# djene-mengistu/UAPS

Measured on AMD Instinct MI355X. Metric: training images/sec (labeled+unlabeled) NEU-Seg 256x256 K=3, higher is better.
Workload: dtype f32

## Files before the change

### uaps_amd/csrc/mid_bwd_row.hip

```cpp
#include "../../include/uaps_hip.h"
#include "conv_kernels.hpp"
#include "conv_split.hpp"
#include "hints.hpp"
#include "row_pieces.hpp"

extern "C" int uaps_conv_get_mode(void);
extern "C" unsigned uaps_conv_get_tuning(void);

namespace uaps {

struct MidBwdArgs {
    const float* dact;
    const float* y2;
    const float* coef;
    float dt_slope;
    int dt_Bg;
    const float* y1;
    const float2* xf;
    float slope;
    int Bg;
    const float* wp;
    const float* wscale;
    int CGP;
    float* g;
    float* slab; float* bslab; int nsplit;
    const float* dy_bound; const float* in_bound;
    float dy_mul, in_mul;
    const float* bs_mean; const float* bs_invstd; const float* bs_gamma; const float* bs_beta;
    float2* partials;
    float* bs_max;
    unsigned* err;
    int B, H;
};

__global__ __launch_bounds__(512, 2) void mid_bwd_row_kernel(MidBwdArgs a) {
    using G = RowGeom<16>;
    constexpr int NG = G::NG, ROWS = G::ROWS, CI = G::CI, NTHR = 512, NXL = G::NXL, MW = G::MW, D_UNITS = G::D_UNITS;
    constexpr int RED_FLOATS = 2 * 10 * 256;
    static_assert(RED_FLOATS / 4 <= G::X_UNITS, "the reduction scratch fits the input image");

    __shared__ __attribute__((aligned(16))) u32x4 sX[G::X_UNITS];
    __shared__ __attribute__((aligned(16))) u32x4 sD[2 * D_UNITS];
    __shared__ __attribute__((aligned(16))) u32x4 sIn[2 * G::PIECE];
    __shared__ __attribute__((aligned(16))) float sG[16 * G::GS];

    const f32x2 sd = h16_scale(__builtin_fmaxf(bound_of(a.dy_bound, a.dy_mul), 0.f));
    const f32x2 sx = h16_scale(__builtin_fmaxf(bound_of(a.in_bound, a.in_mul), 0.f));
    const float sc_d = sd.x, inv_d = sd.y, sc_x = sx.x, inv_x = sx.y;

    const int tid = threadIdx.x, lane = tid & 63, wave = tid >> 6;
    const int j = lane & 15, kq = lane >> 4;
    const int wave_u = __builtin_amdgcn_readfirstlane(wave);
    const int HW = a.H * G::WIDTH;
    const uint32_t HW4 = (uint32_t)HW * 4u;

    RowRuns rr;
    if (!row_runs<G>(a.B, a.H, a.nsplit, rr)) return;

    zero_x_halo<G, NTHR>(sX, tid);
    zero_ring_margins<G, NTHR>(sIn, tid);

    float bs_md = 0.f, bs_mx = 0.f;

    if (wave_u < 4) {
        const int sp = wave_u;
        const int dc0 = wave_u * 4, cg = wave_u >> 1, ch = wave_u & 1;
        const bool want_bias = a.bslab != nullptr;
        f32x4 rd[4], ry[4];
        bool d_in = false;
        float dtc[4][6];
        auto load_d = [&](int b, int gy, f32x4 (&dd)[4], f32x4 (&yy)[4], bool& ok) {
            ok = load_rows4<G>(a.dact, b, gy, a.H, dc0, lane, dd);
            load_rows4<G>(a.y2, b, gy, a.H, dc0, lane, yy);
        };
        auto store_d = [&](f32x4 (&dd)[4], f32x4 (&yy)[4], bool ok, int slot, int buf) {
            f32x4 v[4];
#pragma unroll
            for (int i = 0; i < 4; ++i) {
                asm volatile("" : "+v"(dd[i]));
                asm volatile("" : "+v"(yy[i]));
#pragma unroll
                for (int k = 0; k < 4; ++k) {
                    const float g0 = dd[i][k];
                    const float yc = yy[i][k] - dtc[i][0];
                    const float z = yc * dtc[i][2] + dtc[i][3];
                    const float d = z > 0.f ? g0 : g0 * a.dt_slope;
                    const float t = dtc[i][2] * (d - dtc[i][4] - (yc * dtc[i][1]) * dtc[i][5]);
                    v[i][k] = ok ? t : 0.f;
                }
            }
            store_ring_rows<G>(sIn, v, sc_d, cg, ch, lane, slot);
            if (buf >= 0) {
#pragma unroll
                for (int i = 0; i < 4; ++i) {
                    unsigned a0, a1, b0, b1;
                    conv_split2h(v[i][0] * sc_d, v[i][1] * sc_d, a0, a1);
                    conv_split2h(v[i][2] * sc_d, v[i][3] * sc_d, b0, b1);
                    const int c = dc0 + i;
                    *reinterpret_cast<uint2*>(reinterpret_cast<unsigned*>(&sD[buf * D_UNITS + c * NG]) + lane * 2) = make_uint2(a0, b0);
                    *reinterpret_cast<uint2*>(reinterpret_cast<unsigned*>(&sD[buf * D_UNITS + (16 + c) * NG]) + lane * 2) = make_uint2(a1, b1);
                }
            }
        };

        f32x4 acc[9];
        f32x4 accb = f32x4{0.f, 0.f, 0.f, 0.f};
#pragma unroll
        for (int t = 0; t < 9; ++t) acc[t] = f32x4{0.f, 0.f, 0.f, 0.f};

        for (int run = rr.begin; run < rr.end; ++run) {
            const int b = run / rr.rpi, r0 = (run % rr.rpi) * ROWS;
            const int grp2 = b / a.dt_Bg;
#pragma unroll
            for (int i = 0; i < 4; ++i)
#pragma unroll
                for (int k = 0; k < 6; ++k) dtc[i][k] = a.coef[((size_t)grp2 * 16 + dc0 + i) * 8 + k];
            {
                f32x4 da[4], ya[4], db[4], yb[4];
                bool oka, okb;
                load_d(b, r0 - 1, da, ya, oka);
                load_d(b, r0, db, yb, okb);
                load_d(b, r0 + 1, rd, ry, d_in);
                __builtin_amdgcn_sched_barrier(0);
                store_d(da, ya, oka, 0, -1);
                store_d(db, yb, okb, 1, 0);
                store_d(rd, ry, d_in, 2, 1);
            }
            __syncthreads();
            int s0 = 0, buf = 0;
#pragma unroll 1
            for (int t = r0; t < r0 + ROWS; ++t) {
                const bool more = t + 1 < r0 + ROWS;
                if (more) load_d(b, t + 2, rd, ry, d_in);
                int s1, s2;
                ring_slots<G>(s0, s1, s2);
                const auto slot_of = [&](int ky) { return ky == 0 ? s0 : (ky == 1 ? s1 : s2); };
                const u32x4* sDb = sD + buf * D_UNITS;
#pragma unroll
                for (int sgi = 0; sgi < 2; ++sgi) {
                    const int gq = (sp * 2 + sgi) * 4 + kq;
                    f16x8 af[2];
                    read_dy_frag<G>(sDb, j, gq, af);
                    tap_contract<G>(sX, af, j, gq, slot_of, want_bias, acc, accb);
                }
                __syncthreads();
                if (more) store_d(rd, ry, d_in, s0, buf);
                s0 = s1; buf ^= 1;
                __syncthreads();
            }
        }

        ksplit_reduce<1>(reinterpret_cast<float*>(sX), sp, 0, lane, acc, accb);
        if (sp == 0) store_slabs<true>(a.slab, a.bslab, want_bias, rr.split, 16, CI, 0, j, kq, acc, accb, inv_d, inv_x, a.err);
    } else {
        const int wg = wave_u - 4;
        const int xc0 = wg * NXL;
        const float out_scale_a = inv_d, out_scale_w = a.wscale[1];

        GradFrags<G> wf;
        load_grad_frags<G, 16>(wf, a.wp, a.CGP, j, j, kq, wg * MW);

        f32x4 rx[NXL], xa[NXL], xb[NXL];
        BnRowSums<G> bn;
        bool x_in = false;
        auto store_x = [&](f32x4 (&src)[NXL], bool ok, int slot) { store_act_rows<G>(sX, src, bn.cf, ok, a.slope, sc_x, xc0, lane, slot); };

        for (int run = rr.begin; run < rr.end; ++run) {
            const int b = run / rr.rpi, r0 = (run % rr.rpi) * ROWS;
            bn_run_begin(bn, a.xf, a.bs_mean, a.bs_invstd, a.bs_gamma, a.bs_beta, b / a.Bg, xc0);
            {
                f32x4 ra[NXL];
                const bool oka = load_rows4<G>(a.y1, b, r0 - 1, a.H, xc0, lane, ra);
                const bool okb = load_rows4<G>(a.y1, b, r0, a.H, xc0, lane, xa);
                x_in = load_rows4<G>(a.y1, b, r0 + 1, a.H, xc0, lane, xb);
                __builtin_amdgcn_sched_barrier(0);
                store_x(ra, oka, 0);
                store_x(xa, okb, 1);
                store_x(xb, x_in, 2);
            }
            __syncthreads();
            int s0 = 0;
            const __amdgpu_buffer_rsrc_t rs_g = make_rsrc(a.g + (size_t)b * CI * HW, (uint32_t)CI * HW4);
#pragma unroll 1
            for (int t = r0; t < r0 + ROWS; ++t) {
                const bool more = t + 1 < r0 + ROWS;
                if (more) x_in = load_rows4<G>(a.y1, b, t + 2, a.H, xc0, lane, rx);
                int s1, s2;
                ring_slots<G>(s0, s1, s2);

                f32x4 gacc[MW];
#pragma unroll
                for (int m = 0; m < MW; ++m) gacc[m] = f32x4{0.f, 0.f, 0.f, 0.f};
                grad_row_tiles<G>(sIn, wf, s0, s1, s2, gacc);
                put_grad_row<G>(sG, gacc, out_scale_a, out_scale_w, j, kq, wg * MW, a.err);
                __syncthreads();

#pragma unroll
                for (int i = 0; i < NXL; ++i) bn_row(bn, i, take_row_out<G>(sG, rs_g, xc0 + i, t, HW, lane), xa[i], a.slope, bs_md, bs_mx);
                if (more) store_x(rx, x_in, s0);
#pragma unroll
                for (int i = 0; i < NXL; ++i) { xa[i] = xb[i]; xb[i] = rx[i]; }
                s0 = s1;
                __syncthreads();
            }
            bn_run_end(bn, a.partials, a.B, b, rr.rpi, r0 / ROWS, xc0, lane);
        }
        __syncthreads(); __syncthreads(); __syncthreads(); __syncthreads();
    }
    block_amax_to(a.bs_max, bs_md, sG);
    block_amax_to(a.bs_max + UAPS_BOUND_FLOATS, bs_mx, sG + 16);
}

}

extern "C" int uaps_mid_bwd_fused(const float* dact, const float* y2, const float* coef, float slope2, int groups2, const float* y1,
                                  const void* xf, float slope, int groups, const float* wb, const float* dy_bound, float dy_mul,
                                  const float* x_bound, float x_mul, const float* save_mean, const float* save_invstd,
                                  const float* gamma, const float* beta, int want_bias, int B, int Cin, int Cout, int H, int W, int ks,
                                  int cfg, float* g, void* partials, float* maxes, void* ws, size_t ws_bytes, uaps_stream_t stream) {
    if (!dact || !y1 || !xf || !wb || !save_mean || !save_invstd || !gamma || !beta || !g || !partials || !maxes || !ws) return UAPS_EINVAL;
    if (B <= 0 || Cin <= 0 || Cout <= 0 || H <= 0 || W <= 0 || groups < 1 || B % groups || (uintptr_t)xf % 8) return UAPS_EINVAL;
    if ((y2 || coef) && (!y2 || !coef || groups2 < 1 || B % groups2)) return UAPS_EINVAL;
    if (!(slope >= 0.f && slope <= 1.f)) return UAPS_ERANGE;
    if (ks != 3 || Cin != 16 || Cout != 16 || W != 256 || H % 16 || H > 65536 || (cfg & ~0x3ff)) return UAPS_ENOFORM;
    if (!y2 || !coef) return UAPS_ENOFORM;
    if (uaps_conv_get_mode() != 2 || !dy_bound || !x_bound) return UAPS_ENOFORM;
    if (uaps_conv_get_tuning() & (UAPS_TUNE_NO_ROW_WRW | UAPS_TUNE_NO_SPLIT_WRW)) return UAPS_ENOFORM;
    if (((uintptr_t)dact | (uintptr_t)y2 | (uintptr_t)y1 | (uintptr_t)g | (uintptr_t)wb | (uintptr_t)ws | (uintptr_t)coef) % 16) return UAPS_ENOFORM;
    uaps::MidBwdArgs a{};
    const int rc = uaps::row_wrw_bn_args(a, 16, B, Cin, Cout, H, W, ks, cfg, want_bias, ws, ws_bytes, dy_bound, dy_mul, x_bound, x_mul,
                                         save_mean, save_invstd, gamma, beta, partials, maxes);
    if (rc) return rc;
    uaps::account_bytes(4.0 * B * H * W * (3.0 * Cout + 1.0 * Cin));
    a.dact = dact; a.y2 = y2; a.coef = coef; a.dt_slope = slope2; a.dt_Bg = B / groups2;
    a.y1 = y1; a.xf = (const float2*)xf; a.slope = slope; a.Bg = B / groups;
    const uaps::H16BwdWeights w16 = uaps::h16_bwd_weights(wb, Cin, Cout);
    a.wp = w16.wp; a.wscale = w16.wscale; a.CGP = w16.CGP;
    a.g = g;
    a.B = B; a.H = H;
    UAPS_LAUNCH_MAIN(uaps::mid_bwd_row_kernel, dim3(uaps::row_grid(a.nsplit)), dim3(512), 0, (hipStream_t)stream, a);
    return (int)hipGetLastError();
}
```

### uaps_amd/csrc/row_pieces.hpp

```cpp
#pragma once
#include "conv_kernels.hpp"
#include "conv_split.hpp"
#include "hints.hpp"

namespace uaps {

template <int CI_>
struct RowGeom {
    static constexpr int WIDTH = 256, ROWS = 16, NSLOT = 3, CI = CI_;
    static constexpr int NG = WIDTH / 8, XG = NG + 2;
    static constexpr int X_UNITS = 2 * CI * NSLOT * XG;
    static constexpr int D_UNITS = 2 * 16 * NG;
    static constexpr int IW = WIDTH + 8, CGU = NSLOT * IW, PIECE = 2 * CGU, XS = 3;
    static constexpr int NQ = 9 * 2, NSTEP = (NQ + 3) / 4, MW = 4;
    static constexpr int GS = WIDTH + 4;
    static constexpr int NXL = 4;
};

struct RowRuns { int split, rpi, begin, end; };
template <class G>
__device__ __forceinline__ bool row_runs(int B, int H, int nsplit, RowRuns& r) {
    r.split = xcd_swizzle(blockIdx.x, gridDim.x);
    if (r.split >= nsplit) return false;
    r.rpi = H / G::ROWS;
    const int nruns = B * r.rpi;
    r.begin = (int)((long)nruns * r.split / nsplit); r.end = (int)((long)nruns * (r.split + 1) / nsplit);
    return true;
}
template <class G>
__device__ __forceinline__ void ring_slots(int s0, int& s1, int& s2) {
    s1 = s0 + 1 >= G::NSLOT ? s0 + 1 - G::NSLOT : s0 + 1; s2 = s1 + 1 >= G::NSLOT ? s1 + 1 - G::NSLOT : s1 + 1;
}
template <class G, int NTHR>
__device__ __forceinline__ void zero_x_halo(u32x4* sX, int tid) {
    for (int e = tid; e < 2 * G::CI * G::NSLOT * 2; e += NTHR) sX[(e / 2) * G::XG + (e % 2) * (G::XG - 1)] = u32x4{0u, 0u, 0u, 0u};
}
template <class G, int NTHR>
__device__ __forceinline__ void zero_ring_margins(u32x4* sIn, int tid) {
    for (int e = tid; e < 2 * 2 * G::NSLOT * 8; e += NTHR) sIn[(e / 8) * G::IW + (e % 8 < 4 ? e % 8 : G::IW - 8 + e % 8)] = u32x4{0u, 0u, 0u, 0u};
}

template <class G>
__device__ __forceinline__ bool load_rows4(const float* t, int b, int gy, int H, int c0, int lane, f32x4 (&dst)[4]) {
    const int HW = H * G::WIDTH;
    const uint32_t HW4 = (uint32_t)HW * 4u;
    const bool ok = (unsigned)gy < (unsigned)H;
    const __amdgpu_buffer_rsrc_t rs = make_rsrc(t + (size_t)b * 16 * HW, 16u * HW4);
    const uint32_t off = (uint32_t)(c0 * HW + gy * G::WIDTH + lane * 4) * 4u;
#pragma unroll
    for (int i = 0; i < 4; ++i) dst[i] = __builtin_bit_cast(f32x4, __builtin_amdgcn_raw_buffer_load_b128(rs, (int)(ok ? off + (uint32_t)i * HW4 : kOob), 0, 0));
    return ok;
}

template <class G, class SlotOf>
__device__ __forceinline__ void tap_contract(const u32x4* sX, const f16x8 (&af)[2], int ci, int gq, const SlotOf& slot_of, bool bias,
                                             f32x4 (&acc)[9], f32x4& accb) {
    constexpr unsigned kOnes = 0x3C003C00u;
    const f16x8 ones = __builtin_bit_cast(f16x8, u32x4{kOnes, kOnes, kOnes, kOnes});
    if (bias) {
        accb = __builtin_amdgcn_mfma_f32_16x16x32_f16(af[1], ones, accb, 0, 0, 0);
        accb = __builtin_amdgcn_mfma_f32_16x16x32_f16(af[0], ones, accb, 0, 0, 0);
    }
#pragma unroll
    for (int ky = 0; ky < 3; ++ky) {
        const int slot = slot_of(ky);
        f16x8 bf[3][2];
#pragma unroll
        for (int p = 0; p < 2; ++p) {
            const int u = ((p * G::CI + ci) * G::NSLOT + slot) * G::XG + gq + 1;
            const u32x4 c = sX[u];
            const unsigned cl3 = reinterpret_cast<const unsigned*>(&sX[u - 1])[3];
            const unsigned cr0 = reinterpret_cast<const unsigned*>(&sX[u + 1])[0];
            const unsigned t01 = __builtin_amdgcn_alignbit(c[1], c[0], 16), t12 = __builtin_amdgcn_alignbit(c[2], c[1], 16);
            const unsigned t23 = __builtin_amdgcn_alignbit(c[3], c[2], 16);
            const unsigned tE0 = __builtin_amdgcn_alignbit(c[0], cl3, 16), t3E = __builtin_amdgcn_alignbit(cr0, c[3], 16);
            bf[0][p] = __builtin_bit_cast(f16x8, u32x4{tE0, t01, t12, t23});
            bf[1][p] = __builtin_bit_cast(f16x8, c);
            bf[2][p] = __builtin_bit_cast(f16x8, u32x4{t01, t12, t23, t3E});
        }
#pragma unroll
        for (int kx = 0; kx < 3; ++kx) {
            f32x4 c = acc[ky * 3 + kx];
            c = __builtin_amdgcn_mfma_f32_16x16x32_f16(af[1], bf[kx][0], c, 0, 0, 0);
            c = __builtin_amdgcn_mfma_f32_16x16x32_f16(af[0], bf[kx][1], c, 0, 0, 0);
            c = __builtin_amdgcn_mfma_f32_16x16x32_f16(af[0], bf[kx][0], c, 0, 0, 0);
            acc[ky * 3 + kx] = c;
        }
    }
}
template <class G>
__device__ __forceinline__ void read_dy_frag(const u32x4* sD, int j, int gq, f16x8 (&af)[2]) {
#pragma unroll
    for (int p = 0; p < 2; ++p) af[p] = __builtin_bit_cast(f16x8, sD[(p * 16 + j) * G::NG + gq]);
}

template <int WCI>
__device__ __forceinline__ void ksplit_reduce(float* red, int sp, int wci, int lane, f32x4 (&acc)[9], f32x4& accb) {
#pragma unroll
    for (int s = 2; s >= 1; s >>= 1) {
        if (sp >= s && sp < 2 * s) {
            float* p = red + (size_t)((sp - s) * WCI + wci) * 10 * 256 + lane;
#pragma unroll
            for (int t = 0; t < 9; ++t)
#pragma unroll
                for (int r = 0; r < 4; ++r) p[(t * 4 + r) * 64] = acc[t][r];
#pragma unroll
            for (int r = 0; r < 4; ++r) p[(36 + r) * 64] = accb[r];
        }
        __syncthreads();
        if (sp < s) {
            const float* p = red + (size_t)(sp * WCI + wci) * 10 * 256 + lane;
#pragma unroll
            for (int t = 0; t < 9; ++t)
#pragma unroll
                for (int r = 0; r < 4; ++r) acc[t][r] += p[(t * 4 + r) * 64];
#pragma unroll
            for (int r = 0; r < 4; ++r) accb[r] += p[(36 + r) * 64];
        }
        __syncthreads();
    }
}

template <bool PIN = false>
__device__ __forceinline__ void store_slabs(float* slab, float* bslab, bool bias, int split, int CoutS, int CinS, int ci0, int j, int kq,
                                            const f32x4 (&acc)[9], const f32x4& accb, float inv_d, float inv_x, unsigned* err) {
    slab += (size_t)split * 9 * CoutS * CinS;
    float chk = 0.f;
    const float inv = inv_d * inv_x;
#pragma unroll
    for (int t = 0; t < 9; ++t) {
        note_nonfinite(chk, acc[t]);
#pragma unroll
        for (int r = 0; r < 4; ++r) {
            const int co = kq * 4 + r, ci = ci0 + j;
            if (co < CoutS && ci < CinS) slab[((size_t)t * CoutS + co) * CinS + ci] = acc[t][r] * inv;
        }
    }
    report_nonfinite(err, chk, UAPS_ERR_WRW_NONFINITE);
    if (bias && j == 0) {
        float inv_b = inv_d;
        if constexpr (PIN) asm volatile("" : "+v"(inv_b));
#pragma unroll
        for (int r = 0; r < 4; ++r)
            if (kq * 4 + r < CoutS) bslab[(size_t)split * CoutS + kq * 4 + r] = accb[r] * inv_b;
    }
}

template <class G>
struct BnRowSums {
    f32x2 cf[G::NXL];
    float mu[G::NXL], is[G::NXL], sc[G::NXL], sh[G::NXL];
    float st_s[G::NXL][4], st_q[G::NXL][4];
};

template <class G>
__device__ __forceinline__ void store_act_rows(u32x4* sX, f32x4 (&src)[G::NXL], const f32x2 (&cf)[G::NXL], bool ok, float slope, float sc_x,
                                               int xc0, int lane, int slot) {
#pragma unroll
    for (int i = 0; i < G::NXL; ++i) {
        asm volatile("" : "+v"(src[i]));
        float v[4];
#pragma unroll
        for (int k = 0; k < 4; ++k) {
            const float z = __builtin_fmaf(src[i][k], cf[i].x, cf[i].y);
            v[k] = ok ? __builtin_fmaxf(z, z * slope) : 0.f;
        }
        unsigned a0, a1, b0, b1;
        conv_split2h(v[0] * sc_x, v[1] * sc_x, a0, a1);
        conv_split2h(v[2] * sc_x, v[3] * sc_x, b0, b1);
        const int c = xc0 + i;
        unsigned* p0 = reinterpret_cast<unsigned*>(&sX[(c * G::NSLOT + slot) * G::XG + 1]) + lane * 2;
        unsigned* p1 = reinterpret_cast<unsigned*>(&sX[((G::CI + c) * G::NSLOT + slot) * G::XG + 1]) + lane * 2;
        *reinterpret_cast<uint2*>(p0) = make_uint2(a0, b0);
        *reinterpret_cast<uint2*>(p1) = make_uint2(a1, b1);
    }
}

template <class G>
__device__ __forceinline__ void store_ring_rows(u32x4* sIn, const f32x4 (&v)[4], float scale, int cg, int ch, int lane, int slot) {
    const int base = (cg * G::NSLOT + slot) * G::IW + 4 + lane * 4;
#pragma unroll
    for (int k = 0; k < 4; ++k) {
        unsigned q00, q01, q10, q11;
        conv_split2h(v[0][k] * scale, v[1][k] * scale, q00, q01);
        conv_split2h(v[2][k] * scale, v[3][k] * scale, q10, q11);
        *reinterpret_cast<uint2*>(reinterpret_cast<unsigned*>(&sIn[base + k]) + ch * 2) = make_uint2(q00, q10);
        *reinterpret_cast<uint2*>(reinterpret_cast<unsigned*>(&sIn[G::PIECE + base + k]) + ch * 2) = make_uint2(q01, q11);
    }
}

template <class G>
struct GradFrags {
    u32x4 bfr[G::NSTEP][2];
    int kxo[G::NSTEP], kyv[G::NSTEP], abase[G::MW];
};
template <class G, int CoutP>
__device__ __forceinline__ void load_grad_frags(GradFrags<G>& f, const float* wp, int CGP, int co, int j, int kq, int tile0) {
    const __amdgpu_buffer_rsrc_t rs_w = make_rsrc(wp, (uint32_t)(2 * 9) * CGP * CoutP * 16u);
#pragma unroll
    for (int s = 0; s < G::NSTEP; ++s) {
        const int q = 4 * s + kq, tap = q / 2, cgq = q % 2;
#pragma unroll
        for (int p = 0; p < 2; ++p) {
            const uint32_t off = q < G::NQ ? (uint32_t)(((p * 9 + tap) * CGP + cgq) * CoutP + co) * 16u : kOob;
            f.bfr[s][p] = __builtin_amdgcn_raw_buffer_load_b128(rs_w, (int)off, 0, 0);
        }
        const int qq = q < G::NQ ? q : 0;
        f.kxo[s] = (qq % 2) * G::CGU + (qq / 2) % 3; f.kyv[s] = (qq / 2) / 3;
    }
#pragma unroll
    for (int m = 0; m < G::MW; ++m) f.abase[m] = (tile0 + m) * 16 + j + G::XS;
}

template <class G>
__device__ __forceinline__ void grad_row_tiles(const u32x4* sIn, const GradFrags<G>& f, int s0, int s1, int s2, f32x4 (&gacc)[G::MW]) {
    constexpr int NSTEP = G::NSTEP, MW = G::MW;
    int aoff[NSTEP];
#pragma unroll
    for (int s = 0; s < NSTEP; ++s) aoff[s] = f.kxo[s] + (f.kyv[s] == 0 ? s0 : (f.kyv[s] == 1 ? s1 : s2)) * G::IW;
    constexpr int NUN = NSTEP * MW;
    u32x4 af[2][2];
    auto read_a = [&](int u, u32x4 (&dst)[2]) {
        const int s = u / MW, m = u % MW;
#pragma unroll
        for (int p = 0; p < 2; ++p) dst[p] = sIn[p * G::PIECE + f.abase[m] + aoff[s]];
    };
    read_a(0, af[0]);
#pragma unroll
    for (int u = 0; u < NUN; ++u) {
        const int s = u / MW, m = u % MW;
        if (u + 1 < NUN) read_a(u + 1, af[(u + 1) & 1]);
        const auto Hf = [](const u32x4& v) { return __builtin_bit_cast(f16x8, v); };
        f32x4 c = gacc[m];
        c = __builtin_amdgcn_mfma_f32_16x16x32_f16(Hf(af[u & 1][1]), Hf(f.bfr[s][0]), c, 0, 0, 0);
        c = __builtin_amdgcn_mfma_f32_16x16x32_f16(Hf(af[u & 1][0]), Hf(f.bfr[s][1]), c, 0, 0, 0);
        c = __builtin_amdgcn_mfma_f32_16x16x32_f16(Hf(af[u & 1][0]), Hf(f.bfr[s][0]), c, 0, 0, 0);
        gacc[m] = c;
        if (u + 1 < NUN) __builtin_amdgcn_sched_group_barrier(0x100, 2, 0);
        __builtin_amdgcn_sched_group_barrier(0x008, 3, 0);
    }
}
template <class G>
__device__ __forceinline__ void put_grad_row(float* sG, const f32x4 (&gacc)[G::MW], float out_scale_a, float out_scale_w, int j, int kq,
                                             int tile0, unsigned* err) {
    float chk = 0.f;
#pragma unroll
    for (int m = 0; m < G::MW; ++m) {
        f32x4 v = gacc[m];
        v *= out_scale_a; v *= out_scale_w;
        v += 0.f;
        note_nonfinite(chk, v);
        *reinterpret_cast<f32x4*>(&sG[j * G::GS + (tile0 + m) * 16 + kq * 4]) = v;
    }
    report_nonfinite(err, chk, UAPS_ERR_CONV_NONFINITE);
}
template <class G>
__device__ __forceinline__ f32x4 take_row_out(const float* sG, __amdgpu_buffer_rsrc_t rs_g, int c, int t, int HW, int lane) {
    const f32x4 gv = *reinterpret_cast<const f32x4*>(&sG[c * G::GS + lane * 4]);
    __builtin_amdgcn_raw_buffer_store_b128(__builtin_bit_cast(u32x4, gv), rs_g, (int)((uint32_t)(c * HW + t * G::WIDTH + lane * 4) * 4u), 0, 0);
    return gv;
}

template <class G>
__device__ __forceinline__ void bn_run_begin(BnRowSums<G>& s, const float2* xf, const float* mean, const float* invstd, const float* gamma,
                                             const float* beta, int grp, int xc0) {
#pragma unroll
    for (int i = 0; i < G::NXL; ++i) {
        const int c = xc0 + i;
        const float2 t = xf[(size_t)grp * G::CI + c];
        s.cf[i] = f32x2{t.x, t.y};
        s.mu[i] = mean[grp * G::CI + c]; s.is[i] = invstd[grp * G::CI + c];
        s.sc[i] = gamma[c] * s.is[i]; s.sh[i] = beta[c];
#pragma unroll
        for (int v = 0; v < 4; ++v) { s.st_s[i][v] = 0.f; s.st_q[i][v] = 0.f; }
    }
}
template <class G>
__device__ __forceinline__ void bn_row(BnRowSums<G>& s, int i, const f32x4& gv, const f32x4& yv, float slope, float& md, float& mx) {
    float cs = s.st_s[i][0], cq = s.st_q[i][0];
#pragma unroll
    for (int e = 0; e < 4; ++e) {
        const float yc = yv[e] - s.mu[i], z = yc * s.sc[i] + s.sh[i];
        const float d = z > 0.f ? gv[e] : gv[e] * slope, xh = yc * s.is[i];
        cs += d; cq += d * xh;
        md = __builtin_fmaxf(md, __builtin_fabsf(d)); mx = __builtin_fmaxf(mx, __builtin_fabsf(xh));
    }
#pragma unroll
    for (int v = 0; v < 3; ++v) { s.st_s[i][v] = s.st_s[i][v + 1]; s.st_q[i][v] = s.st_q[i][v + 1]; }
    s.st_s[i][3] = cs; s.st_q[i][3] = cq;
}
template <class G>
__device__ __forceinline__ void bn_run_end(const BnRowSums<G>& st, float2* partials, int B, int b, int rpi, int ri, int xc0, int lane) {
#pragma unroll
    for (int i = 0; i < G::NXL; ++i) {
        float s = 0.f, q = 0.f;
#pragma unroll
        for (int v = 0; v < 4; ++v) {
            float sv = st.st_s[i][v], qv = st.st_q[i][v];
#pragma unroll
            for (int o = 32; o > 0; o >>= 1) { sv += __shfl_xor(sv, o, 64); qv += __shfl_xor(qv, o, 64); }
            s = v == 0 ? sv : s + sv; q = v == 0 ? qv : q + qv;
        }
        if (lane == 0) partials[((size_t)(xc0 + i) * B + b) * rpi + ri] = make_float2(s, q);
    }
}

inline unsigned row_grid(int nsplit) { return (unsigned)((nsplit + 7) / 8 * 8); }

template <class Args>
inline int row_wrw_bn_args(Args& a, int CoutS, int B, int Cin, int Cout, int H, int W, int ks, int cfg, int want_bias, void* ws, size_t ws_bytes,
                           const float* dy_bound, float dy_mul, const float* x_bound, float x_mul, const float* save_mean,
                           const float* save_invstd, const float* gamma, const float* beta, void* partials, float* maxes) {
    size_t need = 0;
    const int rc = uaps_conv_wrw_workspace_bytes(B, Cin, Cout, H, W, ks, cfg, &need);
    if (rc) return rc;
    constexpr int CinS = 16;
    const size_t per_split = ((size_t)9 * CoutS * CinS + CoutS) * sizeof(float);
    if (need == 0 || need % per_split) return UAPS_ENOFORM;
    if (ws_bytes < need) return UAPS_EWORKSPACE;
    a.nsplit = (int)(need / per_split);
    a.slab = (float*)ws;
    a.bslab = want_bias ? a.slab + (size_t)a.nsplit * 9 * CoutS * CinS : nullptr;
    a.dy_bound = dy_bound; a.dy_mul = dy_mul; a.in_bound = x_bound; a.in_mul = x_mul;
    a.bs_mean = save_mean; a.bs_invstd = save_invstd; a.bs_gamma = gamma; a.bs_beta = beta;
    a.partials = (float2*)partials; a.bs_max = maxes;
    a.err = error_word();
    return UAPS_OK;
}

}
```

### uaps_amd/csrc/up_bwd_row.hip

```cpp
#include "../../include/uaps_hip.h"
#include "conv_kernels.hpp"
#include "conv_split.hpp"
#include "hints.hpp"
#include "row_pieces.hpp"
#include "up2_staging.hpp"

extern "C" int uaps_conv_get_mode(void);
extern "C" unsigned uaps_conv_get_tuning(void);

namespace uaps {

typedef unsigned u32x2 __attribute__((ext_vector_type(2)));

struct UpBwdArgs {
    const float* dy;
    const float* wp;
    const float* wscale;
    int CGP;
    float* dskip;
    float* dlow;
    const float* dy_bound; float dy_mul;
    float rh, rw;
    unsigned* err;
    int B, H, nsplit;
};

__device__ __forceinline__ float up_fold_weight(float r, int o, int n_out, int n_in, int i) {
    if (o < 0 || o >= n_out) return 0.f;
    const float sx = mul_rn(r, (float)o);
    const int i0 = (int)sx, i1 = i0 + (i0 < n_in - 1 ? 1 : 0);
    const float l1 = sx - (float)i0, l0 = 1.f - l1;
    return (i0 == i ? l0 : 0.f) + (i1 == i ? l1 : 0.f);
}

__global__ __launch_bounds__(512, 2) void up_bwd_row_kernel(UpBwdArgs a) {
    using G = RowGeom<16>;
    constexpr int WIDTH = G::WIDTH, ROWS = G::ROWS, NTHR = 512, NCH = 4, MW = G::MW, CoutP = 32, GS = G::GS;

    __shared__ __attribute__((aligned(16))) u32x4 sIn[2 * G::PIECE];
    __shared__ __attribute__((aligned(16))) float sG[2][16 * GS];

    const f32x2 sc = h16_scale(__builtin_fmaxf(bound_of(a.dy_bound, a.dy_mul), 0.f));
    const float in_scale = sc.x, out_scale_a = sc.y, out_scale_w = a.wscale[1];

    const int tid = threadIdx.x, lane = tid & 63, wave = tid >> 6;
    const int j = lane & 15, kq = lane >> 4;
    const int wave_u = __builtin_amdgcn_readfirstlane(wave);
    const bool is_up = wave_u >= 4;
    const int half = wave_u >> 2, wq = wave_u & 3;
    const int W = WIDTH, HW = a.H * W, h = a.H / 2, w = WIDTH / 2;
    const uint32_t HW4 = (uint32_t)HW * 4u, hw4 = (uint32_t)(h * w) * 4u;

    RowRuns rr;
    if (!row_runs<G>(a.B, a.H, a.nsplit, rr)) return;

    zero_ring_margins<G, NTHR>(sIn, tid);

    GradFrags<G> wf;
    load_grad_frags<G, CoutP>(wf, a.wp, a.CGP, half * 16 + j, j, kq, wq * MW);

    const int dc0 = wq * NCH, cg = wq >> 1, ch = wq & 1;
    f32x4 rd[NCH];
    auto load_d = [&](int b, int gy, f32x4 (&dd)[NCH]) { load_rows4<G>(a.dy, b, gy, a.H, dc0, lane, dd); };
    auto store_d = [&](f32x4 (&dd)[NCH], int slot) {
#pragma unroll
        for (int i = 0; i < NCH; ++i) asm volatile("" : "+v"(dd[i]));
        store_ring_rows<G>(sIn, dd, in_scale, cg, ch, lane, slot);
    };

    float wxa[4], wxb[4];
#pragma unroll
    for (int k = 0; k < 4; ++k) {
        wxa[k] = up_fold_weight(a.rw, 4 * lane - 1 + k, W, w, 2 * lane);
        wxb[k] = up_fold_weight(a.rw, 4 * lane + 1 + k, W, w, 2 * lane + 1);
    }
    float accp[NCH][2], accq[NCH][2];
#pragma unroll
    for (int i = 0; i < NCH; ++i) { accp[i][0] = accp[i][1] = 0.f; accq[i][0] = accq[i][1] = 0.f; }

    for (int run = rr.begin; run < rr.end; ++run) {
        const int b = run / rr.rpi, r0 = (run % rr.rpi) * ROWS;
        if (!is_up) {
            f32x4 da[NCH], db[NCH];
            load_d(b, r0 - 2, da);
            load_d(b, r0 - 1, db);
            load_d(b, r0, rd);
            __builtin_amdgcn_sched_barrier(0);
            store_d(da, 0);
            store_d(db, 1);
            store_d(rd, 2);
        }
        __syncthreads();
        int s0 = 0;
        const __amdgpu_buffer_rsrc_t rs_g = make_rsrc(a.dskip + (size_t)b * 16 * HW, 16u * HW4);
        const __amdgpu_buffer_rsrc_t rs_l = make_rsrc(a.dlow + (size_t)b * 16 * h * w, 16u * hw4);
#pragma unroll 1
        for (int t = r0 - 1; t <= r0 + ROWS; ++t) {
            const bool more = t < r0 + ROWS;
            if (!is_up && more) load_d(b, t + 2, rd);
            int s1, s2;
            ring_slots<G>(s0, s1, s2);
            const bool own = t >= r0 && t < r0 + ROWS;
            const bool work = is_up ? (unsigned)t < (unsigned)a.H : own;

            f32x4 gacc[MW];
#pragma unroll
            for (int m = 0; m < MW; ++m) gacc[m] = f32x4{0.f, 0.f, 0.f, 0.f};
            if (work) grad_row_tiles<G>(sIn, wf, s0, s1, s2, gacc);
            put_grad_row<G>(sG[half], gacc, out_scale_a, out_scale_w, j, kq, wq * MW, a.err);
            __syncthreads();

            if (!is_up) {
                if (own) {
#pragma unroll
                    for (int i = 0; i < NCH; ++i) take_row_out<G>(sG[0], rs_g, dc0 + i, t, HW, lane);
                }
                if (more) store_d(rd, s0);
            } else {
                const bool odd = (t & 1) != 0;
                const int ip = odd ? (t - 1) / 2 : t / 2 - 1, iq = ip + 1;
                const float wyp = up_fold_weight(a.rh, t, a.H, h, ip), wyq = up_fold_weight(a.rh, t, a.H, h, iq);
                const bool out = !odd && t > r0;
#pragma unroll
                for (int i = 0; i < NCH; ++i) {
                    const f32x4 gv = *reinterpret_cast<const f32x4*>(&sG[1][(dc0 + i) * GS + lane * 4]);
                    const float prev = up2_lane_prev(gv[3]), next = up2_lane_next(gv[0]);
                    float ta = mul_rn(wxa[0], prev);
                    ta = add_rn(ta, mul_rn(wxa[1], gv[0])); ta = add_rn(ta, mul_rn(wxa[2], gv[1])); ta = add_rn(ta, mul_rn(wxa[3], gv[2]));
                    float tb = mul_rn(wxb[0], gv[1]);
                    tb = add_rn(tb, mul_rn(wxb[1], gv[2])); tb = add_rn(tb, mul_rn(wxb[2], gv[3])); tb = add_rn(tb, mul_rn(wxb[3], next));
                    accp[i][0] = add_rn(accp[i][0], mul_rn(wyp, ta)); accp[i][1] = add_rn(accp[i][1], mul_rn(wyp, tb));
                    if (odd) { accq[i][0] = mul_rn(wyq, ta); accq[i][1] = mul_rn(wyq, tb); }
                    else { accq[i][0] = add_rn(accq[i][0], mul_rn(wyq, ta)); accq[i][1] = add_rn(accq[i][1], mul_rn(wyq, tb)); }
                    if (!odd) {
                        const f32x2 lo = f32x2{accp[i][0], accp[i][1]};
                        __builtin_amdgcn_raw_buffer_store_b64(__builtin_bit_cast(u32x2, lo), rs_l,
                                                              (int)(out ? (uint32_t)((dc0 + i) * h * w + ip * w + lane * 2) * 4u : kOob), 0, 0);
                        accp[i][0] = accq[i][0]; accp[i][1] = accq[i][1];
                    }
                }
            }
            s0 = s1;
            __syncthreads();
        }
    }
}

}

namespace {
void fold_support(int n_in, int* lo, int* hi) {
    const int n_out = 2 * n_in;
    const float r = n_out > 1 ? (float)(n_in - 1) / (float)(n_out - 1) : 0.f;
    int mn = n_out, mx = -n_out;
    for (int o = 0; o < n_out; ++o) {
        volatile float sx = r * (float)o;
        const float s = sx;
        const int i0 = (int)s, i1 = i0 + (i0 < n_in - 1 ? 1 : 0);
        volatile float l1v = s - (float)i0;
        const float l1 = l1v;
        volatile float l0v = 1.f - l1;
        const float l0 = l0v;
        const int is[2] = {i0, i1};
        const float ws[2] = {i0 == i1 ? l0 + l1 : l0, i0 == i1 ? 0.f : l1};
        for (int k = 0; k < 2; ++k) {
            if (ws[k] == 0.f) continue;
            const int d = o - 2 * is[k];
            if (d < mn) mn = d;
            if (d > mx) mx = d;
        }
    }
    *lo = mn; *hi = mx;
}
}

extern "C" int uaps_up_fold_support(int n_in, int* min_offset, int* max_offset) {
    if (n_in <= 0 || n_in > (1 << 20) || !min_offset || !max_offset) return UAPS_EINVAL;
    fold_support(n_in, min_offset, max_offset);
    return UAPS_OK;
}

extern "C" int uaps_up_bwd_fused_form(int H, int W) {
    if (H <= 0 || W <= 0) return UAPS_EINVAL;
    if (W != 256 || H % 16 || H > 65536) return UAPS_ENOFORM;
    int lo = 0, hi = 0;
    fold_support(H / 2, &lo, &hi);
    if (lo < -1 || hi > 2) return UAPS_ENOFORM;
    fold_support(W / 2, &lo, &hi);
    if (lo < -1 || hi > 2) return UAPS_ENOFORM;
    return UAPS_OK;
}

extern "C" int uaps_up_bwd_fused_grid(int B, int H) {
    if (B <= 0 || H <= 0 || H % 16) return UAPS_EINVAL;
    const long nruns = (long)B * (H / 16);
    return (int)(nruns < 256 ? nruns : 256);
}

extern "C" int uaps_up_bwd_fused(const float* dy, const float* wb, const float* dy_bound, float dy_mul, float* dskip, int C1, float* dlow,
                                 int C2, int B, int Cout, int H, int W, int ks, int cfg, uaps_stream_t stream) {
    if (!dy || !wb || !dskip || !dlow) return UAPS_EINVAL;
    if (B <= 0 || C1 <= 0 || C2 <= 0 || Cout <= 0 || H <= 0 || W <= 0) return UAPS_EINVAL;
    if (ks != 3 || Cout != 16 || C1 != 16 || C2 != 16 || W != 256 || H % 16 || H > 65536 || (cfg & ~UAPS_CONV_BOUNDED)) return UAPS_ENOFORM;
    if ((long)B * (H / 16) > 0x7fffffffL) return UAPS_ENOFORM;
    if (uaps_conv_get_mode() != 2 || !dy_bound) return UAPS_ENOFORM;
    if (uaps_conv_get_tuning() & (UAPS_TUNE_NO_SPLIT_FWD | UAPS_TUNE_NO_HP16 | UAPS_TUNE_NO_ROW16)) return UAPS_ENOFORM;
    if (((uintptr_t)dy | (uintptr_t)wb | (uintptr_t)dskip | (uintptr_t)dlow) % 16) return UAPS_ENOFORM;
    const int rc = uaps_up_bwd_fused_form(H, W);
    if (rc) return rc;
    uaps::account_bytes(4.0 * B * H * W * (1.0 * Cout + 1.0 * C1 + 0.25 * C2));
    uaps::UpBwdArgs a{};
    a.dy = dy;
    const uaps::H16BwdWeights w16 = uaps::h16_bwd_weights(wb, C1 + C2, Cout);
    a.wp = w16.wp; a.wscale = w16.wscale; a.CGP = w16.CGP;
    a.dskip = dskip; a.dlow = dlow;
    a.dy_bound = dy_bound; a.dy_mul = dy_mul;
    a.rh = (float)(H / 2 - 1) / (float)(H - 1); a.rw = (float)(W / 2 - 1) / (float)(W - 1);
    a.err = uaps::error_word();
    a.B = B; a.H = H;
    a.nsplit = uaps_up_bwd_fused_grid(B, H);
    UAPS_LAUNCH_MAIN(uaps::up_bwd_row_kernel, dim3(uaps::row_grid(a.nsplit)), dim3(512), 0, (hipStream_t)stream, a);
    return (int)hipGetLastError();
}
```

Measured before the change: 2782.

## Merge consecutive row runs per image and share A-fragments across both output halves

Row runs that belong to the same image are now walked as one continuous strip, so the halo rows are loaded and synchronized once per strip instead of once per 16-row run. BN partial sums are still flushed every 16 rows to keep the per-run partials layout. In the upsample backward kernel, each wave now computes both 16-channel output halves over two tiles, reusing each LDS A-fragment read for two MFMAs instead of splitting the halves across wave groups. The change also switches one BN accumulation to explicit rounded mul/add, which may alter codegen. It adds register pressure from doubled weight fragments and accumulators.

```diff
diff --git a/uaps_amd/csrc/mid_bwd_row.hip b/uaps_amd/csrc/mid_bwd_row.hip
--- a/uaps_amd/csrc/mid_bwd_row.hip
+++ b/uaps_amd/csrc/mid_bwd_row.hip
@@ -108,8 +108,10 @@
 #pragma unroll
         for (int t = 0; t < 9; ++t) acc[t] = f32x4{0.f, 0.f, 0.f, 0.f};
 
-        for (int run = rr.begin; run < rr.end; ++run) {
-            const int b = run / rr.rpi, r0 = (run % rr.rpi) * ROWS;
+        for (int run = rr.begin; run < rr.end;) {
+            const RowWalk wk = row_walk<G>(rr, run);
+            const int b = wk.b, r0 = wk.r0, r1 = wk.r1;
+            run += wk.nrun;
             const int grp2 = b / a.dt_Bg;
 #pragma unroll
             for (int i = 0; i < 4; ++i)
@@ -129,8 +131,8 @@
             __syncthreads();
             int s0 = 0, buf = 0;
 #pragma unroll 1
-            for (int t = r0; t < r0 + ROWS; ++t) {
-                const bool more = t + 1 < r0 + ROWS;
+            for (int t = r0; t < r1; ++t) {
+                const bool more = t + 1 < r1;
                 if (more) load_d(b, t + 2, rd, ry, d_in);
                 int s1, s2;
                 ring_slots<G>(s0, s1, s2);
@@ -165,8 +167,10 @@
         bool x_in = false;
         auto store_x = [&](f32x4 (&src)[NXL], bool ok, int slot) { store_act_rows<G>(sX, src, bn.cf, ok, a.slope, sc_x, xc0, lane, slot); };
 
-        for (int run = rr.begin; run < rr.end; ++run) {
-            const int b = run / rr.rpi, r0 = (run % rr.rpi) * ROWS;
+        for (int run = rr.begin; run < rr.end;) {
+            const RowWalk wk = row_walk<G>(rr, run);
+            const int b = wk.b, r0 = wk.r0, r1 = wk.r1;
+            run += wk.nrun;
             bn_run_begin(bn, a.xf, a.bs_mean, a.bs_invstd, a.bs_gamma, a.bs_beta, b / a.Bg, xc0);
             {
                 f32x4 ra[NXL];
@@ -182,17 +186,17 @@
             int s0 = 0;
             const __amdgpu_buffer_rsrc_t rs_g = make_rsrc(a.g + (size_t)b * CI * HW, (uint32_t)CI * HW4);
 #pragma unroll 1
-            for (int t = r0; t < r0 + ROWS; ++t) {
-                const bool more = t + 1 < r0 + ROWS;
+            for (int t = r0; t < r1; ++t) {
+                const bool more = t + 1 < r1;
                 if (more) x_in = load_rows4<G>(a.y1, b, t + 2, a.H, xc0, lane, rx);
                 int s1, s2;
                 ring_slots<G>(s0, s1, s2);
 
-                f32x4 gacc[MW];
-#pragma unroll
-                for (int m = 0; m < MW; ++m) gacc[m] = f32x4{0.f, 0.f, 0.f, 0.f};
+                f32x4 gacc[1][MW];
+#pragma unroll
+                for (int m = 0; m < MW; ++m) gacc[0][m] = f32x4{0.f, 0.f, 0.f, 0.f};
                 grad_row_tiles<G>(sIn, wf, s0, s1, s2, gacc);
-                put_grad_row<G>(sG, gacc, out_scale_a, out_scale_w, j, kq, wg * MW, a.err);
+                put_grad_row<G>(sG, gacc[0], out_scale_a, out_scale_w, j, kq, wg * MW, a.err);
                 __syncthreads();
 
 #pragma unroll
@@ -200,10 +204,13 @@
                 if (more) store_x(rx, x_in, s0);
 #pragma unroll
                 for (int i = 0; i < NXL; ++i) { xa[i] = xb[i]; xb[i] = rx[i]; }
+                if ((t & (ROWS - 1)) == ROWS - 1) {
+                    bn_run_end(bn, a.partials, a.B, b, rr.rpi, t / ROWS, xc0, lane);
+                    bn_run_reset(bn);
+                }
                 s0 = s1;
                 __syncthreads();
             }
-            bn_run_end(bn, a.partials, a.B, b, rr.rpi, r0 / ROWS, xc0, lane);
         }
         __syncthreads(); __syncthreads(); __syncthreads(); __syncthreads();
     }
diff --git a/uaps_amd/csrc/row_pieces.hpp b/uaps_amd/csrc/row_pieces.hpp
--- a/uaps_amd/csrc/row_pieces.hpp
+++ b/uaps_amd/csrc/row_pieces.hpp
@@ -2,6 +2,7 @@
 #include "conv_kernels.hpp"
 #include "conv_split.hpp"
 #include "hints.hpp"
+#include "rn_math.hpp"
 
 namespace uaps {
 
@@ -27,6 +28,16 @@
     r.begin = (int)((long)nruns * r.split / nsplit); r.end = (int)((long)nruns * (r.split + 1) / nsplit);
     return true;
 }
+struct RowWalk { int b, ri, nrun, r0, r1; };
+template <class G>
+__device__ __forceinline__ RowWalk row_walk(const RowRuns& r, int run) {
+    RowWalk w;
+    w.b = run / r.rpi; w.ri = run % r.rpi;
+    const int left = r.end - run, in_image = r.rpi - w.ri;
+    w.nrun = left < in_image ? left : in_image;
+    w.r0 = w.ri * G::ROWS; w.r1 = w.r0 + w.nrun * G::ROWS;
+    return w;
+}
 template <class G>
 __device__ __forceinline__ void ring_slots(int s0, int& s1, int& s2) {
     s1 = s0 + 1 >= G::NSLOT ? s0 + 1 - G::NSLOT : s0 + 1; s2 = s1 + 1 >= G::NSLOT ? s1 + 1 - G::NSLOT : s1 + 1;
@@ -189,63 +200,66 @@
     }
 }
 
-template <class G>
+template <class G, int NH = 1, int MT = G::MW>
 struct GradFrags {
-    u32x4 bfr[G::NSTEP][2];
-    int kxo[G::NSTEP], kyv[G::NSTEP], abase[G::MW];
+    u32x4 bfr[NH][G::NSTEP][2];
+    int kxo[G::NSTEP], kyv[G::NSTEP], abase[MT];
 };
-template <class G, int CoutP>
-__device__ __forceinline__ void load_grad_frags(GradFrags<G>& f, const float* wp, int CGP, int co, int j, int kq, int tile0) {
+template <class G, int CoutP, int NH, int MT>
+__device__ __forceinline__ void load_grad_frags(GradFrags<G, NH, MT>& f, const float* wp, int CGP, int co, int j, int kq, int tile0) {
     const __amdgpu_buffer_rsrc_t rs_w = make_rsrc(wp, (uint32_t)(2 * 9) * CGP * CoutP * 16u);
 #pragma unroll
     for (int s = 0; s < G::NSTEP; ++s) {
         const int q = 4 * s + kq, tap = q / 2, cgq = q % 2;
 #pragma unroll
-        for (int p = 0; p < 2; ++p) {
-            const uint32_t off = q < G::NQ ? (uint32_t)(((p * 9 + tap) * CGP + cgq) * CoutP + co) * 16u : kOob;
-            f.bfr[s][p] = __builtin_amdgcn_raw_buffer_load_b128(rs_w, (int)off, 0, 0);
-        }
+        for (int hf = 0; hf < NH; ++hf)
+#pragma unroll
+            for (int p = 0; p < 2; ++p) {
+                const uint32_t off = q < G::NQ ? (uint32_t)(((p * 9 + tap) * CGP + cgq) * CoutP + co + hf * 16) * 16u : kOob;
+                f.bfr[hf][s][p] = __builtin_amdgcn_raw_buffer_load_b128(rs_w, (int)off, 0, 0);
+            }
         const int qq = q < G::NQ ? q : 0;
         f.kxo[s] = (qq % 2) * G::CGU + (qq / 2) % 3; f.kyv[s] = (qq / 2) / 3;
     }
 #pragma unroll
-    for (int m = 0; m < G::MW; ++m) f.abase[m] = (tile0 + m) * 16 + j + G::XS;
-}
-
-template <class G>
-__device__ __forceinline__ void grad_row_tiles(const u32x4* sIn, const GradFrags<G>& f, int s0, int s1, int s2, f32x4 (&gacc)[G::MW]) {
-    constexpr int NSTEP = G::NSTEP, MW = G::MW;
+    for (int m = 0; m < MT; ++m) f.abase[m] = (tile0 + m) * 16 + j + G::XS;
+}
+
+template <class G, int H0 = 0, int NH, int MT>
+__device__ __forceinline__ void grad_row_tiles(const u32x4* sIn, const GradFrags<G, NH, MT>& f, int s0, int s1, int s2, f32x4 (&gacc)[NH][MT]) {
+    constexpr int NSTEP = G::NSTEP;
     int aoff[NSTEP];
 #pragma unroll
     for (int s = 0; s < NSTEP; ++s) aoff[s] = f.kxo[s] + (f.kyv[s] == 0 ? s0 : (f.kyv[s] == 1 ? s1 : s2)) * G::IW;
-    constexpr int NUN = NSTEP * MW;
+    constexpr int NUN = NSTEP * MT;
     u32x4 af[2][2];
     auto read_a = [&](int u, u32x4 (&dst)[2]) {
-        const int s = u / MW, m = u % MW;
+        const int s = u / MT, m = u % MT;
 #pragma unroll
         for (int p = 0; p < 2; ++p) dst[p] = sIn[p * G::PIECE + f.abase[m] + aoff[s]];
     };
     read_a(0, af[0]);
 #pragma unroll
     for (int u = 0; u < NUN; ++u) {
-        const int s = u / MW, m = u % MW;
+        const int s = u / MT, m = u % MT;
         if (u + 1 < NUN) read_a(u + 1, af[(u + 1) & 1]);
         const auto Hf = [](const u32x4& v) { return __builtin_bit_cast(f16x8, v); };
-        f32x4 c = gacc[m];
-        c = __builtin_amdgcn_mfma_f32_16x16x32_f16(Hf(af[u & 1][1]), Hf(f.bfr[s][0]), c, 0, 0, 0);
-        c = __builtin_amdgcn_mfma_f32_16x16x32_f16(Hf(af[u & 1][0]), Hf(f.bfr[s][1]), c, 0, 0, 0);
-        c = __builtin_amdgcn_mfma_f32_16x16x32_f16(Hf(af[u & 1][0]), Hf(f.bfr[s][0]), c, 0, 0, 0);
-        gacc[m] = c;
+#pragma unroll
+        for (int hf = H0; hf < NH; ++hf) gacc[hf][m] = __builtin_amdgcn_mfma_f32_16x16x32_f16(Hf(af[u & 1][1]), Hf(f.bfr[hf][s][0]), gacc[hf][m], 0, 0, 0);
+#pragma unroll
+        for (int hf = H0; hf < NH; ++hf) gacc[hf][m] = __builtin_amdgcn_mfma_f32_16x16x32_f16(Hf(af[u & 1][0]), Hf(f.bfr[hf][s][1]), gacc[hf][m], 0, 0, 0);
+#pragma unroll
+        for (int hf = H0; hf < NH; ++hf) gacc[hf][m] = __builtin_amdgcn_mfma_f32_16x16x32_f16(Hf(af[u & 1][0]), Hf(f.bfr[hf][s][0]), gacc[hf][m], 0, 0, 0);
         if (u + 1 < NUN) __builtin_amdgcn_sched_group_barrier(0x100, 2, 0);
-        __builtin_amdgcn_sched_group_barrier(0x008, 3, 0);
-    }
-}
-template <class G>
-__device__ __forceinline__ void put_grad_row(float* sG, const f32x4 (&gacc)[G::MW], float out_scale_a, float out_scale_w, int j, int kq,
+        __builtin_amdgcn_sched_group_barrier(0x008, 3 * (NH - H0), 0);
+    }
+}
+template <class G, int MT>
+__device__ __forceinline__ void put_grad_row(float* sG, const f32x4 (&gacc)[MT], float out_scale_a, float out_scale_w, int j, int kq,
                                              int tile0, unsigned* err) {
     float chk = 0.f;
 #pragma unroll
-    for (int m = 0; m < G::MW; ++m) {
+    for (int m = 0; m < MT; ++m) {
         f32x4 v = gacc[m];
         v *= out_scale_a; v *= out_scale_w;
         v += 0.f;
@@ -261,6 +275,13 @@
     return gv;
 }
 
+template <class G>
+__device__ __forceinline__ void bn_run_reset(BnRowSums<G>& s) {
+#pragma unroll
+    for (int i = 0; i < G::NXL; ++i)
+#pragma unroll
+        for (int v = 0; v < 4; ++v) { s.st_s[i][v] = 0.f; s.st_q[i][v] = 0.f; }
+}
 template <class G>
 __device__ __forceinline__ void bn_run_begin(BnRowSums<G>& s, const float2* xf, const float* mean, const float* invstd, const float* gamma,
                                              const float* beta, int grp, int xc0) {
@@ -271,9 +292,8 @@
         s.cf[i] = f32x2{t.x, t.y};
         s.mu[i] = mean[grp * G::CI + c]; s.is[i] = invstd[grp * G::CI + c];
         s.sc[i] = gamma[c] * s.is[i]; s.sh[i] = beta[c];
-#pragma unroll
-        for (int v = 0; v < 4; ++v) { s.st_s[i][v] = 0.f; s.st_q[i][v] = 0.f; }
-    }
+    }
+    bn_run_reset(s);
 }
 template <class G>
 __device__ __forceinline__ void bn_row(BnRowSums<G>& s, int i, const f32x4& gv, const f32x4& yv, float slope, float& md, float& mx) {
@@ -282,7 +302,7 @@
     for (int e = 0; e < 4; ++e) {
         const float yc = yv[e] - s.mu[i], z = yc * s.sc[i] + s.sh[i];
         const float d = z > 0.f ? gv[e] : gv[e] * slope, xh = yc * s.is[i];
-        cs += d; cq += d * xh;
+        cs += d; cq = add_rn(cq, mul_rn(d, xh));
         md = __builtin_fmaxf(md, __builtin_fabsf(d)); mx = __builtin_fmaxf(mx, __builtin_fabsf(xh));
     }
 #pragma unroll
diff --git a/uaps_amd/csrc/up_bwd_row.hip b/uaps_amd/csrc/up_bwd_row.hip
--- a/uaps_amd/csrc/up_bwd_row.hip
+++ b/uaps_amd/csrc/up_bwd_row.hip
@@ -35,7 +35,7 @@
 
 __global__ __launch_bounds__(512, 2) void up_bwd_row_kernel(UpBwdArgs a) {
     using G = RowGeom<16>;
-    constexpr int WIDTH = G::WIDTH, ROWS = G::ROWS, NTHR = 512, NCH = 4, MW = G::MW, CoutP = 32, GS = G::GS;
+    constexpr int WIDTH = G::WIDTH, NTHR = 512, NCH = 4, MT = 2, CoutP = 32, GS = G::GS;
 
     __shared__ __attribute__((aligned(16))) u32x4 sIn[2 * G::PIECE];
     __shared__ __attribute__((aligned(16))) float sG[2][16 * GS];
@@ -47,7 +47,7 @@
     const int j = lane & 15, kq = lane >> 4;
     const int wave_u = __builtin_amdgcn_readfirstlane(wave);
     const bool is_up = wave_u >= 4;
-    const int half = wave_u >> 2, wq = wave_u & 3;
+    const int wq = wave_u & 3;
     const int W = WIDTH, HW = a.H * W, h = a.H / 2, w = WIDTH / 2;
     const uint32_t HW4 = (uint32_t)HW * 4u, hw4 = (uint32_t)(h * w) * 4u;
 
@@ -56,8 +56,8 @@
 
     zero_ring_margins<G, NTHR>(sIn, tid);
 
-    GradFrags<G> wf;
-    load_grad_frags<G, CoutP>(wf, a.wp, a.CGP, half * 16 + j, j, kq, wq * MW);
+    GradFrags<G, 2, MT> wf;
+    load_grad_frags<G, CoutP>(wf, a.wp, a.CGP, j, j, kq, wave_u * MT);
 
     const int dc0 = wq * NCH, cg = wq >> 1, ch = wq & 1;
     f32x4 rd[NCH];
@@ -78,8 +78,10 @@
 #pragma unroll
     for (int i = 0; i < NCH; ++i) { accp[i][0] = accp[i][1] = 0.f; accq[i][0] = accq[i][1] = 0.f; }
 
-    for (int run = rr.begin; run < rr.end; ++run) {
-        const int b = run / rr.rpi, r0 = (run % rr.rpi) * ROWS;
+    for (int run = rr.begin; run < rr.end;) {
+        const RowWalk wk = row_walk<G>(rr, run);
+        const int b = wk.b, r0 = wk.r0, r1 = wk.r1;
+        run += wk.nrun;
         if (!is_up) {
             f32x4 da[NCH], db[NCH];
             load_d(b, r0 - 2, da);
@@ -95,19 +97,22 @@
         const __amdgpu_buffer_rsrc_t rs_g = make_rsrc(a.dskip + (size_t)b * 16 * HW, 16u * HW4);
         const __amdgpu_buffer_rsrc_t rs_l = make_rsrc(a.dlow + (size_t)b * 16 * h * w, 16u * hw4);
 #pragma unroll 1
-        for (int t = r0 - 1; t <= r0 + ROWS; ++t) {
-            const bool more = t < r0 + ROWS;
+        for (int t = r0 - 1; t <= r1; ++t) {
+            const bool more = t < r1;
             if (!is_up && more) load_d(b, t + 2, rd);
             int s1, s2;
             ring_slots<G>(s0, s1, s2);
-            const bool own = t >= r0 && t < r0 + ROWS;
-            const bool work = is_up ? (unsigned)t < (unsigned)a.H : own;
-
-            f32x4 gacc[MW];
-#pragma unroll
-            for (int m = 0; m < MW; ++m) gacc[m] = f32x4{0.f, 0.f, 0.f, 0.f};
-            if (work) grad_row_tiles<G>(sIn, wf, s0, s1, s2, gacc);
-            put_grad_row<G>(sG[half], gacc, out_scale_a, out_scale_w, j, kq, wq * MW, a.err);
+            const bool own = t >= r0 && t < r1, inside = (unsigned)t < (unsigned)a.H;
+
+            f32x4 gacc[2][MT];
+#pragma unroll
+            for (int hf = 0; hf < 2; ++hf)
+#pragma unroll
+                for (int m = 0; m < MT; ++m) gacc[hf][m] = f32x4{0.f, 0.f, 0.f, 0.f};
+            if (own) grad_row_tiles<G>(sIn, wf, s0, s1, s2, gacc);
+            else if (inside) grad_row_tiles<G, 1>(sIn, wf, s0, s1, s2, gacc);
+            if (own) put_grad_row<G>(sG[0], gacc[0], out_scale_a, out_scale_w, j, kq, wave_u * MT, a.err);
+            put_grad_row<G>(sG[1], gacc[1], out_scale_a, out_scale_w, j, kq, wave_u * MT, a.err);
             __syncthreads();
 
             if (!is_up) {
```

New measurement: 2781. No clear change (-0.0%).
